# TinyMPC/tinympc-matlab

Hardware: AMD Instinct MI355X
Metric: ADMM iterations/s, batched quadrotor nx=12 nu=4 N=50 (instance-iterations/s, whole job) (higher is better)
Workload: dtype f64

## Files before the change

### __graft_entry__.py

```python
from __future__ import annotations

import hashlib
import importlib.util
import os
import re
import shutil
import subprocess
import sys

ROOT = os.path.dirname(os.path.abspath(__file__))
if ROOT not in sys.path:
    sys.path.insert(0, ROOT)
PKG_DIR = os.path.join(ROOT, "tinympc-matlab_amd")
PKG_NAME = "tinympc_matlab_amd"
CSRC = os.path.join(PKG_DIR, "csrc")
HIP_LIB = os.path.join(PKG_DIR, "libtinympc_hip.so")
ORACLE_DIR = os.path.join(ROOT, "oracle")
REFERENCE_SRC = "/root/reference/src/codegen_src"

HIP_SOURCES = ["tinympc_kernels.hip", "tinympc_precompute_rows.hip", "tinympc_solve.hip", "tinympc_solve_b.hip", "tinympc_solve_fam.hip", "tinympc_solve_adapt.hip", "tinympc_imod_a.hip", "tinympc_ifam_a.hip", "tinympc_solve_c.hip", "tinympc_solve_d.hip", "tinympc_solve_dr.hip", "tinympc_lean_d.hip", "tinympc_lstart_d.hip", "tinympc_ltrim_d.hip", "tinympc_solve_dw.hip", "tinympc_solve_dx.hip", "tinympc_jit.hip", "tinympc_solve_m.hip", "tinympc_precompute_large.hip", "tinympc_handle.hip", "tinympc_plan.hip", "tinympc_session.hip", "tinympc_capi.hip",
               "tinympc_codegen.hip"]
HIP_LINTED = ["tinympc_precompute_rows.hip", "tinympc_solve.hip", "tinympc_solve_b.hip", "tinympc_solve_fam.hip", "tinympc_solve_adapt.hip", "tinympc_imod_a.hip", "tinympc_ifam_a.hip",
              "tinympc_solve_c.hip", "tinympc_solve_d.hip", "tinympc_solve_dr.hip", "tinympc_lean_d.hip", "tinympc_lstart_d.hip", "tinympc_ltrim_d.hip", "tinympc_solve_dw.hip", "tinympc_solve_dx.hip"]
JIT_EMBEDDED = ["tinympc_device.h", "tinympc_sweep.h", "tinympc_fam_red.h", "tinympc_solve_d_chain.h", "tinympc_solve_dw_chain.h", "tinympc_solve_dx_chain.h",
                "tinympc_solve_e_common.h", "tinympc_solve_dwide.h", "tinympc_solve_d.hip", "tinympc_solve_dw.hip", "tinympc_solve_dx.hip", "tinympc_solve_e.hip",
                "tinympc_solve_f.hip"]
_ROCKET = ["-DTINY_JIT_NX=6", "-DTINY_JIT_NU=3", "-DTINY_JIT_N=100", "-DTINY_JIT_CT=0", "-DTINY_JIT_FAM=1"]
_ROCKET_FAM = ["-DTINY_JIT_E_NROUND=1", "-DTINY_JIT_E_NCONE=2", "-DTINY_JIT_E_CONES={0,0,2},{0,6,8}", "-DTINY_JIT_E_NLX=1", "-DTINY_JIT_E_NLU=0"]
HIP_BUILTINS = [
    ("k_builtin_e_rocket100", "tinympc_solve_e.hip",
     _ROCKET + ["-DTINY_JIT_E_WPG=8", "-DTINY_JIT_E_WPS=2", "-DTINY_JIT_E_S=13"] + _ROCKET_FAM +
     ["-DTINY_JIT_E_GC_LDS=0", "-DTINY_JIT_E_GL_LDS=0", "-DTINY_JIT_E_LX_LDS=0", "-DTINY_JIT_E_KFAM=1", "-DTINY_JIT_E_DREG=1"]),
    ("k_builtin_f_rocket100", "tinympc_solve_f.hip", _ROCKET + ["-DTINY_JIT_F_WPG=4", "-DTINY_JIT_F_S=7"] + _ROCKET_FAM + ["-DTINY_JIT_F_KFAM=1"]),
    ("k_builtin_f_rocket100_session", "tinympc_solve_f.hip", _ROCKET + ["-DTINY_JIT_F_WPG=4", "-DTINY_JIT_F_S=7"] + _ROCKET_FAM + ["-DTINY_JIT_F_KFAM=1", "-DTINY_JIT_F_SESSION=1"]),
]
_NO_FAM = ["-DTINY_JIT_E_NROUND=0", "-DTINY_JIT_E_NCONE=0", "-DTINY_JIT_E_CONES={-1,0,0}", "-DTINY_JIT_E_NLX=0", "-DTINY_JIT_E_NLU=0"]
for _name, _nx, _nu, _N, _wpg, _S in (("cartpole20", 4, 1, 20, 2, 3), ("quadrotor50", 12, 4, 50, 4, 4)):
    for _suffix, _ct, _extra in (("", 1, []), ("_var", 0, []), ("_session", 0, ["-DTINY_JIT_F_SESSION=1"])):
        HIP_BUILTINS.append(("k_builtin_f_%s%s" % (_name, _suffix), "tinympc_solve_f.hip",
                             ["-DTINY_JIT_NX=%d" % _nx, "-DTINY_JIT_NU=%d" % _nu, "-DTINY_JIT_N=%d" % _N, "-DTINY_JIT_CT=%d" % _ct, "-DTINY_JIT_FAM=0",
                              "-DTINY_JIT_F_WPG=%d" % _wpg, "-DTINY_JIT_F_S=%d" % _S] + _NO_FAM + _extra))
HIP_BUILTINS_D = [("k_builtin_d_quadrotor50_models", "tinympc_solve_d.hip",
                   ["-DTINY_JIT_NX=12", "-DTINY_JIT_NU=4", "-DTINY_JIT_N=50", "-DTINY_JIT_VREG=49", "-DTINY_JIT_WPS=1", "-DTINY_JIT_WPG=4",
                    "-DTINY_JIT_CT=1", "-DTINY_JIT_FAM=0", "-DTINY_JIT_ADAPT=0", "-DTINY_JIT_IMOD=1"])]
ALL_BUILTINS = HIP_BUILTINS + HIP_BUILTINS_D
BUILD_DIR = os.path.join(ROOT, "build", "hip")
HIP_CFLAGS = ["--offload-arch=gfx950", "-O3", "-std=c++17", "-fPIC", "-fno-gpu-rdc",
              "-Wall", "-Wno-unused-function", "-I" + os.path.join(ROOT, "include"), "-I" + CSRC, "-I" + BUILD_DIR]
HIP_LDFLAGS = ["--offload-arch=gfx950", "-shared", "-fPIC", "-fno-gpu-rdc", "-lhiprtc"]


def load_package():
    if PKG_NAME in sys.modules:
        return sys.modules[PKG_NAME]
    spec = importlib.util.spec_from_file_location(
        PKG_NAME, os.path.join(PKG_DIR, "__init__.py"), submodule_search_locations=[PKG_DIR])
# ... 292 lines not shown
```

### tinympc-matlab_amd/csrc/tinympc_device.h

```cpp
#pragma once
#ifndef __HIPCC_RTC__
#include <hip/hip_runtime.h>
#endif

namespace tinympc {

__host__ __device__ inline size_t ops_doubles(int W, int KT) { return (size_t)2 * W * KT + 3 * W; }

__host__ __device__ inline size_t table_rows(int N) { return (size_t)N + 2; }

constexpr int V_PAD = 4;
__host__ __device__ inline size_t v_rows(int N) { return (size_t)N + 1 + 2 * V_PAD; }
__host__ __device__ inline size_t tables_doubles(int W, int N) { return 3 * table_rows(N) * W + W; }

#if defined(__HIPCC__) || defined(__HIPCC_RTC__)
__device__ __forceinline__ void host_store(double *p, double v) { __hip_atomic_store(p, v, __ATOMIC_RELAXED, __HIP_MEMORY_SCOPE_SYSTEM); }
#endif

struct PrecomputeParams {
    int nx, nu;
    union { double rho; const double *rho_sys; };
    const double *A, *B, *fdyn, *Qd, *Rd;
    double *Kinf, *Pinf, *Quu_inv, *AmBKt, *APf, *BPf;
    int *info;
// ... 267 lines not shown
    double *rho_inst;
    int batch;
    double rho;
    double *mail;
};
hipError_t launch_setup_init(const SetupInitParams &p, hipStream_t stream);
hipError_t launch_fill_bounds(double *xmin, double *xmax, size_t X, double *umin, double *umax, size_t U, double inf, hipStream_t stream);
hipError_t launch_reset_stats(int *istats, double *dstats, double *rho_inst, int batch, double rho, hipStream_t stream);
size_t lqr_scratch_doubles(int nx, int nu);
size_t precompute_large_scratch_doubles(int nx, int nu);
hipError_t launch_precompute_large(const PrecomputeParams &p, hipStream_t stream);
hipError_t launch_build_operators(const OperatorParams &p, hipStream_t stream);
hipError_t launch_build_tables(const TableParams &p, hipStream_t stream);
hipError_t launch_store_inst_refs(const InstRefStoreParams &p, hipStream_t stream);
hipError_t launch_build_inst_tables(const InstTableParams &p, hipStream_t stream);
hipError_t launch_fill_inst_models(const InstModelFillParams &p, hipStream_t stream);
hipError_t launch_store_inst_diag(const InstDiagParams &p, hipStream_t stream);
hipError_t launch_check_positive(const double *v, int n, int *flag, hipStream_t stream);
hipError_t launch_build_inst_lin(const InstLinParams &p, hipStream_t stream);
hipError_t launch_check_inst_lin(const InstLinParams &p, int *flag, hipStream_t stream);
hipError_t launch_check_ref_steps(const int *steps, int n, int delta, int *flag, hipStream_t stream);
hipError_t launch_advance_ref_steps(int *steps, int n, int delta, hipStream_t stream);
enum class SolveExt { Box, Families, Adaptive, InstRefs, InstBounds, InstModels, InstFamilies };
hipError_t launch_solve_a(const SolveParams &p, SolveExt ext, int W, int KT, size_t lds_bytes, hipStream_t stream);
hipError_t launch_solve_b(const SolveParams &p, int W, int KT, size_t lds_bytes, hipStream_t stream);
size_t solve_b_lds_bytes(int nx, int nu, int N, int W);
constexpr int WAVES_PER_GROUP_B = 4;
bool solve_d_supported(int nx, int nu, int N, bool const_tables);
hipError_t launch_solve_d(const SolveParams &p, hipStream_t stream);
hipError_t launch_solve_d_refill(const SolveParams &p, hipStream_t stream);
hipError_t launch_solve_d_lean(const SolveParams &p, hipStream_t stream);
hipError_t launch_solve_d_lean_start(const SolveParams &p, hipStream_t stream);
hipError_t launch_solve_d_lean_trim(const SolveParams &p, hipStream_t stream);
int solve_d_workgroups(int nu, int N, bool const_tables, int groups);
size_t solve_d_lds_bytes(int nu, int N, bool const_tables);
int solve_d_resident_workgroups(int wpg);
int solve_d_wavefronts_per_workgroup(int nu, int N, bool const_tables);
bool solve_dw_supported(int nx, int nu, int N, bool const_tables);
hipError_t launch_solve_dw(const SolveParams &p, hipStream_t stream);
int solve_dw_workgroups(int nu, int N, int groups);
size_t solve_dw_lds_bytes(int nu, int N);
bool solve_dx_supported(int nx, int nu, int N, bool const_tables);
hipError_t launch_solve_dx(const SolveParams &p, hipStream_t stream);
int solve_dx_workgroups(int nu, int N, int groups);
size_t solve_dx_lds_bytes(int nu, int N);
hipError_t launch_solve_c(const SolveParams &p, int W, int KT, size_t lds_bytes, hipStream_t stream);
hipError_t launch_build_chunk_tables(const ChunkTableParams &p, hipStream_t stream);
size_t f_input_table_doubles(int nu, int S);
hipError_t launch_build_f_input_tables(const ChunkTableParams &p, hipStream_t stream);
void chunk_plan(int N, int *S, int *C, int *Lc);
size_t solve_c_lds_bytes(int nx, int Lc);
size_t solve_c_lds_bytes_refs(int nx, int nu, int N, int Lc);
size_t chunk_table_doubles(int nx, int Lc);
int chunk_ks(int nx);
hipError_t launch_build_adapt(const AdaptTableParams &p, hipStream_t stream);
inline hipError_t ensure_dynamic_lds(const void *fn, size_t bytes, size_t (&cache)[16]) {
    int dev = 0;
    hipError_t e = hipGetDevice(&dev);
    if (e != hipSuccess) return e;
    if (dev >= 0 && dev < 16 && cache[dev] >= bytes) return hipSuccess;
    e = hipFuncSetAttribute(fn, hipFuncAttributeMaxDynamicSharedMemorySize, (int)bytes);
    if (e == hipSuccess && dev >= 0 && dev < 16) cache[dev] = bytes;
    return e;
}

bool solve_m_supported(int nx, int nu);
// ... 32 lines not shown
```

### tinympc-matlab_amd/csrc/tinympc_plan.hip

```cpp
#include <cstring>
#include "tinympc_handle.h"

using namespace tinympc;
using namespace tinympc::host;

namespace {

void arm_completion_flag(tinympc_solver *s, SolveParams &p) {
    if (!p.host_sol) return;
    s->session_seq += 1;
    p.host_seq = (double)s->session_seq;
    s->flag_pending = true;
}

void decide_layout_d_variants(tinympc_solver *s) {
    if (!s->layout_d) return;
    if (s->d_varying < 0 && !s->tables_const()) {
        if (s->W == 16 && !s->d_jit && solve_d_supported(s->nx, s->nu, s->N, false)) {
            s->d_varying = 1;
        } else {
            s->d_varying_jit = solve_jit_supported(s->W, s->nx, s->nu, s->N, false);
            s->d_varying = s->d_varying_jit ? 1 : 0;
        }
    }
// ... 212 lines not shown
    const bool ct = s->tables_const();
    long resident;
    if (jit) resident = solve_jit_resident_wavefronts(s->W, s->nx, s->nu, s->N, ct);
    else {
        const int wpg = solve_d_wavefronts_per_workgroup(s->nu, s->N, ct);
        resident = (long)solve_d_resident_workgroups(wpg) * wpg;
    }
    const bool reachable = s->st.abs_pri_tol > 0.0 && s->st.abs_dua_tol > 0.0;
    if ((long)s->groups <= resident) return false;
    if (!reachable && mode != 1) return false;
    return !jit || solve_jit_refill_supported(s->W, s->nx, s->nu, s->N, ct);
}

static bool lean_applies(const tinympc_solver *s, const LaunchPlan &pl) {
    if (pl.kernel != KernelId::D_COMPILED || s->W != 16 || pl.adaptive || pl.families || s->zero_copy_tick || s->st.max_iter <= 0)
        return false;
    if (pl.inst_models) return false;
    if (refill_applies(s, pl)) return false;
    const char *env = getenv("TINYMPC_LEAN");
    const int mode = env ? atoi(env) : -1;
    if (mode == 0) return false;
    if (mode == 1) return true;
    const bool reachable = s->st.abs_pri_tol > 0.0 && s->st.abs_dua_tol > 0.0;
    return s->st.check_termination != 1 || !reachable;
}
static bool lean_start_applies() {
    const char *env = getenv("TINYMPC_LEAN_START");
    return !env || atoi(env) != 0;
}
static bool lean_trim_applies() {
    const char *env = getenv("TINYMPC_LEAN_TRIM");
    return lean_start_applies() && (!env || atoi(env) != 0);
}
static const char *lean_words(const tinympc_solver *s, const LaunchPlan &pl) {
    return !lean_applies(s, pl) ? "" : lean_trim_applies() ? " lean lds-start trim" : lean_start_applies() ? " lean lds-start" : " lean";
}

int launch(tinympc_solver *s, bool timed) {
    int rc;
    s->flag_pending = false;
    if ((rc = resolve_plan(s))) return rc;
    const LaunchPlan pl = current_plan(s);
    const bool fam = pl.families, adaptive = pl.adaptive;
    if (s->inst.lin && !pl.inst_lin) {
        const char *why = s->layout_m ? "for systems with nx+nu > 64"
                          : s->inst.models ? (s->inst.rho_verb ? "with per-instance models or rho (set_model_batch / set_rho_batch); tinympc_clear_model_batch returns to the shared model and rho"
                                                               : "with per-instance models (set_model_batch); tinympc_clear_model_batch returns to the shared model")
                          : adaptive ? "with adaptive rho"
                                     : "with more cones or rounds of overlapping cones than the generic kernel holds";
        return fail(TINYMPC_ERR_UNSUPPORTED, "per-instance linear constraints (set_linear_constraints_batch) are not supported %s; "
                    "tinympc_set_linear_constraints returns to shared rows", why);
    }
    if (s->inst_tables() && !pl.inst_refs) {
        const bool r = s->inst.refs(), b = s->inst.bounds, m = s->inst.models;
        const char *what[3], *back[3];
        int n = 0;
        if (r) { what[n] = "per-instance references (set_x_ref_batch / set_u_ref_batch)"; back[n++] = "tinympc_set_x_ref / tinympc_set_u_ref return to shared references"; }
        if (b) { what[n] = "per-instance bounds (set_bound_constraints_batch)"; back[n++] = "tinympc_set_bound_constraints returns to shared bounds"; }
        if (m) {
            what[n] = s->inst.rho_verb ? "per-instance models (set_model_batch) with per-instance rho (set_rho_batch)" : "per-instance models (set_model_batch)";
            back[n++] = s->inst.rho_verb ? "tinympc_clear_model_batch returns to the shared model and rho" : "tinympc_clear_model_batch returns to the shared model";
        }
        std::string subj, way;
        for (int i = 0; i < n; ++i) {
            subj += std::string(i == 0 ? "" : i == n - 1 ? " and " : ", ") + what[i];
            way += std::string(i == 0 ? "" : ", ") + back[i];
        }
        return fail(TINYMPC_ERR_UNSUPPORTED, "%s are not supported %s; %s", subj.c_str(),
// ... 68 lines not shown
    }
    p.adapt = s->dadapt; p.rho_inst = s->drho_inst;
    if (pl.inst_lin) { p.ilin = s->inst.lrows; p.ilin_nl = s->inst.lin_nl; }
    if (pl.inst_models) p.rho_inst = s->inst.mrho;
    if (pl.inst_refs) {
        p.iref_lr = pl.kernel == KernelId::A ? s->inst.lr_rows() : s->inst.lrg;
        p.iref_pn = s->inst.pn;
        if (pl.kernel != KernelId::A) p.ibnd = s->inst.bndg;
        else if (pl.inst_bounds) p.ibnd = s->inst.bnd;
    }
    p.rho_min = s->st.adaptive_rho_min; p.rho_max = s->st.adaptive_rho_max; p.rho_clip = s->st.adaptive_rho_enable_clipping;
    const bool kernel_takes_cold = (pl.kernel == KernelId::D_COMPILED || pl.kernel == KernelId::D_JIT) && s->st.max_iter > 0;
    if (s->cold_state && !kernel_takes_cold && (rc = materialize_cold_state(s))) return rc;
    p.cold = s->cold_state ? 1 : 0;
    s->cold_state = false;
    if (s->st.max_iter > 0) s->sol_zero_pending = false;
    else if ((rc = materialize_zero_solution(s))) return rc;
    if (refill_applies(s, pl) && !p.x0_mirror && !p.u0_host && !p.host_sol) {
        if (!s->drefill && (rc = dalloc(s, &s->drefill, 1))) return rc;
        HIP_TRY(hipMemsetAsync(s->drefill, 0, sizeof(int), s->stream));
        p.refill_next = s->drefill;
    }
    if (timed) HIP_TRY(hipEventRecord(s->ev0, s->stream));
    switch (pl.kernel) {
        case KernelId::M:
            p.ctab = s->dctab;
            HIP_TRY(launch_solve_m(p, s->stream));
            break;
        case KernelId::D_JIT:
            HIP_TRY(launch_solve_jit(p, s->W, s->stream, pl.inst_models));
            break;
        case KernelId::D_COMPILED:
            if (lean_applies(s, pl) && !p.x0_mirror && !p.u0_host && !p.refill_next)
                HIP_TRY(lean_trim_applies()    ? launch_solve_d_lean_trim(p, s->stream)
                        : lean_start_applies() ? launch_solve_d_lean_start(p, s->stream)
                                               : launch_solve_d_lean(p, s->stream));
            else HIP_TRY(s->W == 64 ? launch_solve_dx(p, s->stream) : s->W == 32 ? launch_solve_dw(p, s->stream) : launch_solve_d(p, s->stream));
            break;
        case KernelId::E:
            p.ctab = s->dctab_e; p.chunk_len = s->e_chunk_len; p.chunk_count = s->e_wpg; p.chunk_levels = 1;
            HIP_TRY(launch_solve_e(p, s->fs, s->stream));
            break;
        case KernelId::F:
            p.ctab = s->dctab_f; p.ftab = s->dftab; p.chunk_len = s->f_chunk_len; p.chunk_count = s->f_chunks; p.chunk_levels = 4;
            arm_completion_flag(s, p);
            HIP_TRY(launch_solve_f(p, s->f_fs, s->stream));
            break;
        case KernelId::C:
            p.ctab = s->dctab; p.chunk_len = s->chunk_len; p.chunk_count = s->chunk_count; p.chunk_levels = s->chunk_levels;
            arm_completion_flag(s, p);
            HIP_TRY(launch_solve_c(p, s->W, s->KT, s->lds_bytes_c, s->stream));
            break;
        case KernelId::B:
            HIP_TRY(launch_solve_b(p, s->W, s->KT, s->lds_bytes, s->stream));
            break;
        case KernelId::A:
        case KernelId::FAM_A:
        case KernelId::ADAPT_A: {
            const SolveExt ext = pl.kernel == KernelId::FAM_A ? SolveExt::Families : pl.kernel == KernelId::ADAPT_A ? SolveExt::Adaptive
                                 : pl.inst_lin ? SolveExt::InstFamilies : pl.inst_models ? SolveExt::InstModels : pl.inst_bounds ? SolveExt::InstBounds : pl.inst_refs ? SolveExt::InstRefs : SolveExt::Box;
            HIP_TRY(launch_solve_a(p, ext, s->W, s->KT, s->lds_bytes_a, s->stream));
            break;
        }
    }
    if (timed) HIP_TRY(hipEventRecord(s->ev1, s->stream));
    return TINYMPC_OK;
}
// ... 87 lines not shown
```

### tinympc-matlab_amd/csrc/tinympc_solve_d.hip

```cpp
#if defined(TINY_BUILTIN) && !defined(TINY_JIT)
#define TINY_JIT 1
#endif
#ifndef TINY_JIT
#include <atomic>
#endif
#include <type_traits>

#include "tinympc_device.h"
#include "tinympc_sweep.h"

#ifndef TINY_REFILL
#if defined(TINY_JIT_REFILL) && TINY_JIT_REFILL
#define TINY_REFILL 1
#else
#define TINY_REFILL 0
#endif
#endif

#ifndef TINY_LEAN
#define TINY_LEAN 0
#endif
#if TINY_LEAN && (TINY_REFILL || defined(TINY_JIT))
#error "TINY_LEAN: compiled-in plain kernels only"
#endif
#ifndef TINY_LEAN_START
#define TINY_LEAN_START 0
#endif
#if TINY_LEAN_START && !TINY_LEAN
#error "TINY_LEAN_START: a variant of the lean kernels"
#endif
#if TINY_LEAN_START && !defined(TINY_LEAN_NO_LDS_START)
#define TINY_LDS_START 1
#else
#define TINY_LDS_START 0
#endif
#if TINY_LEAN_START && !defined(TINY_LEAN_NO_HOIST)
#define TINY_LEAN_HOIST 1
#else
#define TINY_LEAN_HOIST 0
#endif
#ifndef TINY_LEAN_TRIM
#define TINY_LEAN_TRIM 0
#endif
#if TINY_LEAN_TRIM && !(TINY_LEAN_START && TINY_LEAN_HOIST && TINY_LDS_START)
#error "TINY_LEAN_TRIM: a variant of the lean-start kernels (LDS starts and hoisted control)"
#endif
#if TINY_LEAN_TRIM && !defined(TINY_TRIM_NO_DSTORE)
#define TINY_TRIM_DSTORE 1
#define D_DUMP_DOUBLES(nu) (2 * 4 * (nu))
#else
#define TINY_TRIM_DSTORE 0
#endif

#define TINY_STR2(x) #x
#define TINY_STR(x) TINY_STR2(x)
namespace tinympc {
template <int NX, int NU>
struct DStep;
}

#ifdef TINY_JIT
#define D_NX TINY_JIT_NX
#define D_NU TINY_JIT_NU
#include "tinympc_solve_d_chain.h"
#else
#define D_NX 12
#define D_NU 4
#include "tinympc_solve_d_chain.h"
#define D_NX 4
#define D_NU 1
#include "tinympc_solve_d_chain.h"
#endif

namespace tinympc {

template <int I, int E, class F>
__device__ __forceinline__ void static_for(F &&f) {
    if constexpr (I < E) {
        f(std::integral_constant<int, I>{});
        static_for<I + 1, E>(f);
    }
}

constexpr int D_OPS_DOUBLES = 2 * 16 * 16;
// ... 378 lines not shown
    auto load_ops = [&](const double *src, double (&m)[16]) {
        if constexpr (ADAPT) {
            const double delta = rho - rho0;
            static_for<0, 16>([&](auto K) {
                constexpr int o = (K.value < NXU ? K.value : 0) * 16;
                m[K.value] = fma(delta, src[o + (sAd - sOps)], src[o]);
            });
        } else {
            static_for<0, 16>([&](auto K) { m[K.value] = src[(K.value < NXU ? K.value : 0) * 16]; });
        }
    };
    auto vget = [&](auto S) -> double {
        if constexpr (decltype(S)::value >= VL) return Vr[decltype(S)::value - VL];
        else return sVl[decltype(S)::value * 64];
    };

#ifdef TINY_CLOCK_STAMP
    const unsigned long long ck_t0 = __builtin_amdgcn_s_memtime(), ck_r0 = __builtin_amdgcn_s_memrealtime();
#endif
#ifdef TINY_D_PAD
    asm volatile(".rept " TINY_STR(TINY_D_PAD) "\n\ts_nop 0\n\t.endr" ::: "memory");
#endif
#ifdef TINY_D_LOOP_ALIGN
    asm volatile(".p2align " TINY_STR(TINY_D_LOOP_ALIGN) ::: "memory");
#endif
    const int max_iter = p.max_iter;
#if TINY_TRIM_DSTORE
    unsigned aDw = aD;
#endif
#if TINY_LEAN
    auto iteration = [&](auto LEAN_, const int it) __attribute__((always_inline)) -> bool {
#if TINY_LEAN_HOIST
        constexpr bool LEANI = decltype(LEAN_)::value != 0, CTL_ONLY = decltype(LEAN_)::value == 2, NO_CTL = LEANI && !CTL_ONLY;
#else
        constexpr bool LEANI = decltype(LEAN_)::value;
#endif
#else
    for (int it = 0; max_iter > 0; ++it) {
#endif
        const int it0 = __builtin_amdgcn_readfirstlane(it);
#if TINY_LEAN
        const bool final_round = !LEANI && it0 >= max_iter;
#elif TINY_REFILL
        const bool final_round = REFILL ? false : it0 >= max_iter;
#else
        const bool final_round = it0 >= max_iter;
#endif
#if TINY_LEAN_HOIST
        if constexpr (TWO_PER_SIMD && !CTL_ONLY) fair_share_priority<NS>(it0, simd_slot);
#else
        if constexpr (TWO_PER_SIMD) fair_share_priority<NS>(it0, simd_slot);
#endif
#if TINY_REFILL
        const bool fin = REFILL ? it_done >= max_iter : final_round;
        const bool wb = pending || (fin && active);
#elif TINY_LEAN_HOIST
        const bool wb = NO_CTL ? false : pending || (final_round && active);
#else
        const bool wb = pending || (final_round && active);
#endif
        if (TINY_RARE(__ballot(wb) != 0ull)) {
            int lane_o = lane;
            asm volatile("" : "+v"(lane_o));
            const int r_o = lane_o & 15, j_o = lane_o >> 4;
            const bool x_o = r_o < NX;
#if TINY_REFILL
// ... 160 lines not shown
            const double snew = fmin(hi0, fmax(lo0, s));
#if TINY_LEAN_HOIST
            if constexpr (LEANI) G0 = s;
            else G0 = s - snew;
#else
            G0 = s - snew;
#endif
            pri = is_x ? fabs(x0v - snew) : 0.0;
            dua = is_x ? fabs(V0 - snew) : 0.0;
            if (may && !adapt) {
                const bool bad = !((pri < p.abs_pri_tol) && (dua * rho < p.abs_dua_tol));
#if TINY_REFILL
                may = __builtin_amdgcn_readfirstlane((int)wave_may_converge_d(__ballot(bad), __ballot(REFILL ? chk : active))) != 0;
#else
                may = __builtin_amdgcn_readfirstlane((int)wave_may_converge_d(__ballot(bad), __ballot(active))) != 0;
#endif
            }
#if TINY_REFILL
            if (TINY_RARE(may) && is_x && active) gV1u[REFILL ? row_offset(cur) : (unsigned)lane] = V0;
#else
            if (TINY_RARE(may) && is_x && active) gV1u[(unsigned)lane] = V0;
#endif
            V0 = snew;
        }
        if constexpr (FAM) {
            double gcn, gln;
            (void)families(x0v, GC0, GL0, gcn, gln);
            if (is_x) {
                GC0 = gcn;
                GL0 = gln;
            }
        }
        double xcur = x0v;
        double dcur = lds_read_async<0>(aD), vcur = 0.0;
#if TINY_LEAN
        if constexpr (VL > 0 && !LEANI) vcur = lds_read_async<0>(aV);
#else
        if constexpr (VL > 0) vcur = lds_read_async<0>(aV);
#endif
        double locur = lo_c, hicur = hi_c;
        if constexpr (!CT) {
            locur = lds_read_async<W * 8>(aT);
            hicur = lds_read_async<(TOFF + W) * 8>(aT);
        }
        lds_wait_ops(m);
#if TINY_LDS_START
        double acur = 0.0;
#endif
        auto fstep = [&](auto S) {
            constexpr int q = decltype(S)::value;
            double dn = 0.0, vn = 0.0, lon = lo_c, hin = hi_c;
            if constexpr (q + 1 < NS) dn = lds_read_async<(q + 1) * DS * 8>(aD);
#if TINY_LEAN
            if constexpr (q + 1 < VL && !LEANI) vn = lds_read_async<(q + 1) * 512>(aV);
#else
            if constexpr (q + 1 < VL) vn = lds_read_async<(q + 1) * 512>(aV);
#endif
            if constexpr (!CT && q + 1 < NS) {
                lon = lds_read_async<(q + 2) * W * 8>(aT);
                hin = lds_read_async<(TOFF + (q + 2) * W) * 8>(aT);
            }
#if TINY_LDS_START
            static_assert(K0, "step 0 starts from c0");
            double an = 0.0;
            if constexpr (LEANI && q + 1 < NS) an = lds_read_issued_here<0>(aC);
#endif
            const double xprev = xcur;
            double snew_q;
#if TINY_LEAN
            if constexpr (LEANI) {
                if constexpr (q >= VL) {
                    if constexpr (K0 && q == 0) xcur = Step::fwd_reg0_nores(dcur, m, c0, locur, hicur, G[q], Vr[q - VL]);
#if TINY_LDS_START
                    else xcur = Step::fwd_reg_start(xcur, dcur, m, acur, locur, hicur, G[q], Vr[q - VL]);
#else
                    else xcur = Step::fwd_reg_nores(xcur, dcur, m, cf, locur, hicur, G[q], Vr[q - VL]);
#endif
                    snew_q = Vr[q - VL];
                } else {
                    double vnew;
                    if constexpr (K0 && q == 0) xcur = Step::fwd_lds0_nores(dcur, m, c0, locur, hicur, G[q], vnew);
#if TINY_LDS_START
                    else xcur = Step::fwd_lds_start(xcur, dcur, m, acur, locur, hicur, G[q], vnew);
#else
                    else xcur = Step::fwd_lds_nores(xcur, dcur, m, cf, locur, hicur, G[q], vnew);
#endif
                    lds_write_async<q * 512>(aV, vnew);
                    snew_q = vnew;
                }
            } else
#endif
            if constexpr (q >= VL) {
                if constexpr (K0 && q == 0) xcur = Step::fwd_reg0(dcur, m, c0, locur, hicur, G[q], Vr[q - VL], pri, dua);
                else xcur = Step::fwd_reg(xcur, dcur, m, cf, locur, hicur, G[q], Vr[q - VL], pri, dua);
                snew_q = Vr[q - VL];
            } else {
                double vnew;
                if constexpr (K0 && q == 0) xcur = Step::fwd_lds0(dcur, m, c0, locur, hicur, G[q], vcur, vnew, pri, dua);
                else xcur = Step::fwd_lds(xcur, dcur, m, cf, locur, hicur, G[q], vcur, vnew, pri, dua);
                lds_write_async<q * 512>(aV, vnew);
                snew_q = vnew;
            }
            if constexpr (ADAPT) {
                if (adapt) {
// ... 111 lines not shown
#else
            if (active) {
#endif
                snap_pri = pri;
                snap_dua = dua;
                if constexpr (ADAPT) snap_rho = rho;
                res_valid = true;
                if (conv) {
                    status = 1;
                    active = false;
                    pending = true;
                }
            }
        }

        {
            const unsigned long long wr_d = __ballot(is_u && active);
            load_ops(sMb, m);
            auto lr_of = [&](auto S) -> double {
                double base;
                if constexpr (CT) base = lr_c;
                else base = sTl[2 * TOFF + (S.value + 1) * W];
                if constexpr (FAM) base += LX[S.value];
                return base;
            };
            double px, rcur, rnext, acc;
            {
                double lrT = is_x ? pnref_lin : lr_of(std::integral_constant<int, NS - 1>{});
                if constexpr (FAM) lrT = is_x ? pnref_lin + LX[NS - 1] : lrT;
                const double lr2 = lr_of(std::integral_constant<int, NS - 2>{});
                const double lrmc2 = is_x ? lr2 + cb : cb;
                const double v1 = vget(std::integral_constant<int, NS - 1>{}), v2 = vget(std::integral_constant<int, NS - 2>{});
                double t;
                if constexpr (ADAPT) {
                    asm("v_add_f64 %[t], %[v1], -%[g1]\n\t"
                        "v_fma_f64 %[px], %[nrho], %[t], %[lrT]\n\t"
                        "v_add_f64 %[t], %[v2], -%[g2]\n\t"
                        "v_fma_f64 %[acc], %[rhom], %[t], %[lrmc]\n\t"
                        "v_fma_f64 %[rn], %[nrho], %[t], %[lr]"
                        : [t] "=&v"(t), [px] "=&v"(px), [acc] "=&v"(acc), [rn] "=&v"(rnext)
                        : [v1] "v"(v1), [g1] "v"(G[NS - 1]), [v2] "v"(v2), [g2] "v"(G[NS - 2]), [nrho] "v"(nrho_lin), [lrT] "v"(lrT),
                          [rhom] "v"(rhom_lin), [lrmc] "v"(lrmc2), [lr] "v"(lr2));
                } else if constexpr (FOLD) {
                    asm("v_add_f64 %[t], %[v1], -%[g1]\n\t"
                        "v_fma_f64 %[px], %[sc], %[t], %[lrT]\n\t"
                        "v_add_f64 %[rn], %[v2], -%[g2]\n\t"
                        "v_fma_f64 %[acc], %[rhom], %[rn], %[lrmc]"
                        : [t] "=&v"(t), [px] "=&v"(px), [acc] "=&v"(acc), [rn] "=&v"(rnext)
                        : [v1] "v"(v1), [g1] "v"(G[NS - 1]), [v2] "v"(v2), [g2] "v"(G[NS - 2]), [sc] "v"(is_x ? nrho : 1.0),
                          [lrT] "v"(is_x ? pnref : 0.0), [rhom] "v"(rhom), [lrmc] "v"(lrmc_f));
                } else {
                    asm("v_add_f64 %[t], %[v1], -%[g1]\n\t"
                        "v_fma_f64 %[px], %[nrho], %[t], %[lrT]\n\t"
                        "v_add_f64 %[t], %[v2], -%[g2]\n\t"
                        "v_fma_f64 %[acc], %[rhom], %[t], %[lrmc]\n\t"
                        "v_fma_f64 %[rn], %[nrho], %[t], %[lr]"
                        : [t] "=&v"(t), [px] "=&v"(px), [acc] "=&v"(acc), [rn] "=&v"(rnext)
                        : [v1] "v"(v1), [g1] "v"(G[NS - 1]), [v2] "v"(v2), [g2] "v"(G[NS - 2]), [nrho] "s"(nrho), [lrT] "v"(lrT),
                          [rhom] "v"(rhom), [lrmc] "v"(lrmc2), [lr] "v"(lr2));
                }
                rcur = px;
            }
            auto vreq = [&](auto S) -> double {
                if constexpr (decltype(S)::value >= VL) return Vr[decltype(S)::value - VL];
                else return lds_read_async<decltype(S)::value * 512>(aV);
            };
            double v2cur = vreq(std::integral_constant<int, (NS >= 3 ? NS - 3 : 0)>{});
            lds_wait_ops(m);
#if TINY_LEAN_HOIST
            if constexpr (LEANI) {
                asm volatile("" : "+v"(G0));
                G0 = G0 - V0;
                asm volatile("" ::"v"(G0));
            }
#endif
            static_for<0, NS - 1>([&](auto I) {
                constexpr int s = NS - 1 - I.value;
                constexpr int s2 = s >= 2 ? s - 2 : 0;
                constexpr int s3 = s >= 3 ? s - 3 : 0;
                double v2n = 0.0;
                if constexpr (s >= 2) v2n = vreq(std::integral_constant<int, s3>{});
                const double lr2 = lr_of(std::integral_constant<int, s2>{});
                const double lrmc2 = is_x ? lr2 + cb : cb;
                double a = acc, an, rn;
                if constexpr (ADAPT) Step::bwd_v(a, px, rcur, m, v2cur, G[s2], rhom_lin, lrmc2, nrho_lin, lr2, an, rn);
                else if constexpr (FOLD) Step::bwd_fold(a, px, rcur, m, v2cur, G[s2], rhom, lrmc_f, an, rn);
                else Step::bwd(a, px, rcur, m, v2cur, G[s2], rhom, lrmc2, nrho, lr2, an, rn);
#if TINY_TRIM_DSTORE
                if constexpr (NO_CTL) lds_write_async<s * DS * 8>(aDw, a);
                else lds_write_masked<s * DS * 8>(aD, a, wr_d);
#else
                lds_write_masked<s * DS * 8>(aD, a, wr_d);
#endif
                px = a;
                rcur = rnext;
                rnext = rn;
                acc = an;
                v2cur = v2n;
            });
            {
                double a = acc;
                Step::bwd_last(a, px, rcur, m);
#if TINY_TRIM_DSTORE
                if constexpr (NO_CTL) lds_write_async<0>(aDw, a);
                else lds_write_masked<0>(aD, a, wr_d);
#else
                lds_write_masked<0>(aD, a, wr_d);
#endif
            }
        }
#if TINY_LEAN
        return false;
    };
    const bool reachable = p.abs_pri_tol > 0.0 && p.abs_dua_tol > 0.0;
    const int last_check = ct > 0 ? (max_iter / ct) * ct : 0;
    for (int it = 0; max_iter > 0;) {
        int nres = max_iter + 1;
        if (ct > 0 && reachable) nres = (it / ct + 1) * ct;
        else if (last_check > it) nres = last_check;
        const int lean_end = __builtin_amdgcn_readfirstlane(nres - 1 < max_iter ? nres - 1 : max_iter);
#if TINY_LEAN_HOIST
        if (it < lean_end) {
            if (iteration(std::integral_constant<int, 2>{}, it)) break;
#if TINY_TRIM_DSTORE
            {
                const unsigned long long live = __ballot(active);
                const unsigned lm = (unsigned)(live & 1ull) | (unsigned)((live >> 15) & 2ull) | (unsigned)((live >> 30) & 4ull) | (unsigned)((live >> 45) & 8ull);
                const int first = __builtin_ctz(lm | 16u);
                const int cls = (r / NU) % 3;
                int jt = cls == 0 ? j : (j ^ 2);
                if (((lm >> jt) & 1u) == 0u) jt = first & 3;
                const unsigned dump = lds_addr(sD) + (unsigned)((jt * NU + r % NU) * 8) - (unsigned)((cls == 2 ? 2 : 1) * DS * 8);
                aDw = (is_u && active) ? aD : dump;
            }
#endif
            for (; it < lean_end; ++it) (void)iteration(std::true_type{}, it);
            if (active) it_done = __builtin_amdgcn_readfirstlane(it);
        }
        if (iteration(std::false_type{}, it)) break;
#else
        bool over = false;
        for (; it < lean_end; ++it) {
            if (iteration(std::true_type{}, it)) {
                over = true;
                break;
            }
        }
        if (over || iteration(std::false_type{}, it)) break;
#endif
        ++it;
    }
#else
    }
#endif
    lds_wait();
#ifdef TINY_CLOCK_STAMP
    const unsigned long long ck_t1 = __builtin_amdgcn_s_memtime(), ck_r1 = __builtin_amdgcn_s_memrealtime();
#endif

#if TINY_REFILL
    if constexpr (REFILL) return;
#endif
    if (inst_ok && status == 1 && r < NXU) {
        __builtin_amdgcn_fence(__ATOMIC_RELEASE, "wavefront");
        const int rows = is_x ? N : NS;
        double *const wV = p.V + ((size_t)grp * v_rows(N) + V_PAD) * 64 + lane;
        const double *const wV2 = p.V2 + ((size_t)grp * v_rows(N) + V_PAD) * 64 + lane;
        for (int kn = 0; kn < rows; ++kn) wV[kn * 64] = wV2[kn * 64];
    }

    const double res_px = group_max<W>(is_x ? snap_pri : 0.0), res_pu = group_max<W>(is_u ? snap_pri : 0.0);
    const double rho_res = ADAPT ? snap_rho : rho;
    const double res_dx = group_max<W>(is_x ? snap_dua : 0.0) * rho_res, res_du = group_max<W>(is_u ? snap_dua : 0.0) * rho_res;

#ifdef TINY_CLOCK_STAMP
    if (p.scratch && lane == 0) {
        unsigned long long *ck = reinterpret_cast<unsigned long long *>(p.scratch) + 8 * (size_t)grp;
        ck[0] = ck_t1 - ck_t0;
        ck[1] = ck_r1 - ck_r0;
        ck[2] = ck_barrier - ck_entry;
        ck[3] = ck_r0 - ck_barrier;
        ck[4] = __builtin_amdgcn_s_memrealtime() - ck_r1;
        ck[5] = ck_entry;
        ck[6] = __builtin_amdgcn_s_memrealtime();
        ck[7] = (unsigned long long)__builtin_amdgcn_s_getreg((31 << 11) | 4) | ((unsigned long long)__builtin_amdgcn_s_getreg((3 << 11) | 20) << 32);
    }
#endif
    if (inst_ok && r == 0) {
        if constexpr (ADAPT) p.rho_inst[inst] = rho;
        p.istats[inst * 2 + 0] = it_done;
        p.istats[inst * 2 + 1] = status;
        if (res_valid) {
            p.dstats[inst * 4 + 0] = res_px;
            p.dstats[inst * 4 + 1] = res_dx;
            p.dstats[inst * 4 + 2] = res_pu;
            p.dstats[inst * 4 + 3] = res_du;
        }
    }
}

#if TINY_LEAN
#if TINY_LEAN_TRIM
#define k_admm_solve_d_lean k_admm_solve_d_lean_trim
#define k_admm_solve_d_gbnd_lean k_admm_solve_d_gbnd_lean_trim
#define launch_solve_d_lean launch_solve_d_lean_trim
static_assert(d_vl(4, 50, true, 4) == 25, "quadrotor N=50: 25 slack slots in LDS with four wavefronts per workgroup");
#elif TINY_LEAN_START
#define k_admm_solve_d_lean k_admm_solve_d_lean_start
#define k_admm_solve_d_gbnd_lean k_admm_solve_d_gbnd_lean_start
#define launch_solve_d_lean launch_solve_d_lean_start
static_assert(d_vl(4, 50, true, 4) == 25, "quadrotor N=50: 25 slack slots in LDS with four wavefronts per workgroup");
#endif
template <int NX, int NU, int N, bool CT, int WPG, int VL>
__global__ void __launch_bounds__(64 * WPG) __attribute__((amdgpu_waves_per_eu(2, 2))) k_admm_solve_d_lean(const SolveParams p) {
    extern __shared__ __attribute__((aligned(16))) double smem[];
    k_admm_solve_d_body<NX, NU, N, CT, WPG, VL>(p, smem);
}
template <int NX, int NU, int N, int WPG, int VL>
__global__ void __launch_bounds__(64 * WPG) __attribute__((amdgpu_waves_per_eu(2, 2))) k_admm_solve_d_gbnd_lean(const SolveParams p) {
    extern __shared__ __attribute__((aligned(16))) double smem[];
    k_admm_solve_d_body<NX, NU, N, true, WPG, VL, false, false, true, false, false, true>(p, smem);
}

__host__ __device__ constexpr int d_wpg(int nu, int N, bool ct) { return d_vl(nu, N, ct, 4) >= 0 ? 4 : 8; }

template <int NX, int NU, int N, bool CT>
static hipError_t launch_d_one(const SolveParams &p, hipStream_t stream) {
    constexpr int WPG = d_wpg(NU, N, CT);
    constexpr int VL = d_vl(NU, N, CT, WPG);
    if constexpr (VL < 0) {
        return hipErrorInvalidValue;
    } else {
        constexpr size_t lds = d_lds_bytes(NU, N, CT, WPG, VL);
        static size_t lds_set_l[16] = {0}, lds_set_lgoal[16] = {0};
        const int wgs = (p.groups + WPG - 1) / WPG;
// ... 230 lines not shown
```

Baseline: 1.174 billion.

## Add lean-share kernel variant keeping backward-sweep values in registers across iterations

```diff
diff --git a/__graft_entry__.py b/__graft_entry__.py
--- a/__graft_entry__.py
+++ b/__graft_entry__.py
@@ -18,10 +18,10 @@
 ORACLE_DIR = os.path.join(ROOT, "oracle")
 REFERENCE_SRC = "/root/reference/src/codegen_src"
 
-HIP_SOURCES = ["tinympc_kernels.hip", "tinympc_precompute_rows.hip", "tinympc_solve.hip", "tinympc_solve_b.hip", "tinympc_solve_fam.hip", "tinympc_solve_adapt.hip", "tinympc_imod_a.hip", "tinympc_ifam_a.hip", "tinympc_solve_c.hip", "tinympc_solve_d.hip", "tinympc_solve_dr.hip", "tinympc_lean_d.hip", "tinympc_lstart_d.hip", "tinympc_ltrim_d.hip", "tinympc_solve_dw.hip", "tinympc_solve_dx.hip", "tinympc_jit.hip", "tinympc_solve_m.hip", "tinympc_precompute_large.hip", "tinympc_handle.hip", "tinympc_plan.hip", "tinympc_session.hip", "tinympc_capi.hip",
+HIP_SOURCES = ["tinympc_kernels.hip", "tinympc_precompute_rows.hip", "tinympc_solve.hip", "tinympc_solve_b.hip", "tinympc_solve_fam.hip", "tinympc_solve_adapt.hip", "tinympc_imod_a.hip", "tinympc_ifam_a.hip", "tinympc_solve_c.hip", "tinympc_solve_d.hip", "tinympc_solve_dr.hip", "tinympc_lean_d.hip", "tinympc_lstart_d.hip", "tinympc_ltrim_d.hip", "tinympc_lshare_d.hip", "tinympc_solve_dw.hip", "tinympc_solve_dx.hip", "tinympc_jit.hip", "tinympc_solve_m.hip", "tinympc_precompute_large.hip", "tinympc_handle.hip", "tinympc_plan.hip", "tinympc_session.hip", "tinympc_capi.hip",
                "tinympc_codegen.hip"]
 HIP_LINTED = ["tinympc_precompute_rows.hip", "tinympc_solve.hip", "tinympc_solve_b.hip", "tinympc_solve_fam.hip", "tinympc_solve_adapt.hip", "tinympc_imod_a.hip", "tinympc_ifam_a.hip",
-              "tinympc_solve_c.hip", "tinympc_solve_d.hip", "tinympc_solve_dr.hip", "tinympc_lean_d.hip", "tinympc_lstart_d.hip", "tinympc_ltrim_d.hip", "tinympc_solve_dw.hip", "tinympc_solve_dx.hip"]
+              "tinympc_solve_c.hip", "tinympc_solve_d.hip", "tinympc_solve_dr.hip", "tinympc_lean_d.hip", "tinympc_lstart_d.hip", "tinympc_ltrim_d.hip", "tinympc_lshare_d.hip", "tinympc_solve_dw.hip", "tinympc_solve_dx.hip"]
 JIT_EMBEDDED = ["tinympc_device.h", "tinympc_sweep.h", "tinympc_fam_red.h", "tinympc_solve_d_chain.h", "tinympc_solve_dw_chain.h", "tinympc_solve_dx_chain.h",
                 "tinympc_solve_e_common.h", "tinympc_solve_dwide.h", "tinympc_solve_d.hip", "tinympc_solve_dw.hip", "tinympc_solve_dx.hip", "tinympc_solve_e.hip",
                 "tinympc_solve_f.hip"]
diff --git a/tinympc-matlab_amd/csrc/tinympc_device.h b/tinympc-matlab_amd/csrc/tinympc_device.h
--- a/tinympc-matlab_amd/csrc/tinympc_device.h
+++ b/tinympc-matlab_amd/csrc/tinympc_device.h
@@ -323,6 +323,7 @@
 hipError_t launch_solve_d_lean(const SolveParams &p, hipStream_t stream);
 hipError_t launch_solve_d_lean_start(const SolveParams &p, hipStream_t stream);
 hipError_t launch_solve_d_lean_trim(const SolveParams &p, hipStream_t stream);
+hipError_t launch_solve_d_lean_share(const SolveParams &p, hipStream_t stream);
 int solve_d_workgroups(int nu, int N, bool const_tables, int groups);
 size_t solve_d_lds_bytes(int nu, int N, bool const_tables);
 int solve_d_resident_workgroups(int wpg);
diff --git a/tinympc-matlab_amd/csrc/tinympc_lshare_d.hip b/tinympc-matlab_amd/csrc/tinympc_lshare_d.hip
--- /dev/null
+++ b/tinympc-matlab_amd/csrc/tinympc_lshare_d.hip
@@ -0,0 +1,5 @@
+#define TINY_LEAN 1
+#define TINY_LEAN_START 1
+#define TINY_LEAN_TRIM 1
+#define TINY_LEAN_SHARE 1
+#include "tinympc_solve_d.hip"
diff --git a/tinympc-matlab_amd/csrc/tinympc_plan.hip b/tinympc-matlab_amd/csrc/tinympc_plan.hip
--- a/tinympc-matlab_amd/csrc/tinympc_plan.hip
+++ b/tinympc-matlab_amd/csrc/tinympc_plan.hip
@@ -268,8 +268,16 @@
     const char *env = getenv("TINYMPC_LEAN_TRIM");
     return lean_start_applies() && (!env || atoi(env) != 0);
 }
+static bool lean_share_applies() {
+    const char *env = getenv("TINYMPC_LEAN_SHARE");
+    return lean_trim_applies() && (!env || atoi(env) != 0);
+}
 static const char *lean_words(const tinympc_solver *s, const LaunchPlan &pl) {
-    return !lean_applies(s, pl) ? "" : lean_trim_applies() ? " lean lds-start trim" : lean_start_applies() ? " lean lds-start" : " lean";
+    return !lean_applies(s, pl)   ? ""
+           : lean_share_applies() ? " lean lds-start trim share"
+           : lean_trim_applies()  ? " lean lds-start trim"
+           : lean_start_applies() ? " lean lds-start"
+                                  : " lean";
 }
 
 int launch(tinympc_solver *s, bool timed) {
@@ -404,7 +412,8 @@
             break;
         case KernelId::D_COMPILED:
             if (lean_applies(s, pl) && !p.x0_mirror && !p.u0_host && !p.refill_next)
-                HIP_TRY(lean_trim_applies()    ? launch_solve_d_lean_trim(p, s->stream)
+                HIP_TRY(lean_share_applies()   ? launch_solve_d_lean_share(p, s->stream)
+                        : lean_trim_applies()  ? launch_solve_d_lean_trim(p, s->stream)
                         : lean_start_applies() ? launch_solve_d_lean_start(p, s->stream)
                                                : launch_solve_d_lean(p, s->stream));
             else HIP_TRY(s->W == 64 ? launch_solve_dx(p, s->stream) : s->W == 32 ? launch_solve_dw(p, s->stream) : launch_solve_d(p, s->stream));
diff --git a/tinympc-matlab_amd/csrc/tinympc_solve_d.hip b/tinympc-matlab_amd/csrc/tinympc_solve_d.hip
--- a/tinympc-matlab_amd/csrc/tinympc_solve_d.hip
+++ b/tinympc-matlab_amd/csrc/tinympc_solve_d.hip
@@ -50,6 +50,12 @@
 #define D_DUMP_DOUBLES(nu) (2 * 4 * (nu))
 #else
 #define TINY_TRIM_DSTORE 0
+#endif
+#ifndef TINY_LEAN_SHARE
+#define TINY_LEAN_SHARE 0
+#endif
+#if TINY_LEAN_SHARE && !(TINY_LEAN_TRIM && TINY_TRIM_DSTORE)
+#error "TINY_LEAN_SHARE: a variant of the trimmed lean kernels (with their dstore addresses)"
 #endif
 
 #define TINY_STR2(x) #x
@@ -494,6 +500,9 @@
     auto iteration = [&](auto LEAN_, const int it) __attribute__((always_inline)) -> bool {
 #if TINY_LEAN_HOIST
         constexpr bool LEANI = decltype(LEAN_)::value != 0, CTL_ONLY = decltype(LEAN_)::value == 2, NO_CTL = LEANI && !CTL_ONLY;
+#if TINY_LEAN_SHARE
+        constexpr bool SH_F = decltype(LEAN_)::value >= 3, SH_B = decltype(LEAN_)::value == 3;
+#endif
 #else
         constexpr bool LEANI = decltype(LEAN_)::value;
 #endif
@@ -720,7 +729,12 @@
             }
         }
         double xcur = x0v;
+#if TINY_LEAN_SHARE
+        double dcur = 0.0, vcur = 0.0;
+        if constexpr (!(SH_F && VL == 0)) dcur = lds_read_async<0>(aD);
+#else
         double dcur = lds_read_async<0>(aD), vcur = 0.0;
+#endif
 #if TINY_LEAN
         if constexpr (VL > 0 && !LEANI) vcur = lds_read_async<0>(aV);
 #else
@@ -738,7 +752,11 @@
         auto fstep = [&](auto S) {
             constexpr int q = decltype(S)::value;
             double dn = 0.0, vn = 0.0, lon = lo_c, hin = hi_c;
+#if TINY_LEAN_SHARE
+            if constexpr (q + 1 < NS && !(SH_F && q + 1 >= VL)) dn = lds_read_async<(q + 1) * DS * 8>(aD);
+#else
             if constexpr (q + 1 < NS) dn = lds_read_async<(q + 1) * DS * 8>(aD);
+#endif
 #if TINY_LEAN
             if constexpr (q + 1 < VL && !LEANI) vn = lds_read_async<(q + 1) * 512>(aV);
 #else
@@ -758,6 +776,11 @@
 #if TINY_LEAN
             if constexpr (LEANI) {
                 if constexpr (q >= VL) {
+#if TINY_LEAN_SHARE
+                    if constexpr (SH_F && K0 && q == 0) xcur = Step::fwd_reg0_nores(Vr[q - VL], m, c0, locur, hicur, G[q], Vr[q - VL]);
+                    else if constexpr (SH_F) xcur = Step::fwd_reg_start(xcur, Vr[q - VL], m, acur, locur, hicur, G[q], Vr[q - VL]);
+                    else
+#endif
                     if constexpr (K0 && q == 0) xcur = Step::fwd_reg0_nores(dcur, m, c0, locur, hicur, G[q], Vr[q - VL]);
 #if TINY_LDS_START
                     else xcur = Step::fwd_reg_start(xcur, dcur, m, acur, locur, hicur, G[q], Vr[q - VL]);
@@ -935,6 +958,27 @@
                 const double lrmc2 = is_x ? lr2 + cb : cb;
                 const double v1 = vget(std::integral_constant<int, NS - 1>{}), v2 = vget(std::integral_constant<int, NS - 2>{});
                 double t;
+#if TINY_LEAN_SHARE
+                static_assert(NVR >= 3, "the first three slots of the backward sweep are register slots");
+                if constexpr (SH_B && FOLD) {
+                    asm("v_add_f64 %[t], %[acc], -%[g1]\n\t"
+                        "v_fma_f64 %[px], %[sc], %[t], %[lrT]\n\t"
+                        "v_add_f64 %[rn], %[v2], -%[g2]\n\t"
+                        "v_fma_f64 %[acc], %[rhom], %[rn], %[lrmc]"
+                        : [t] "=&v"(t), [px] "=&v"(px), [acc] "+v"(Vr[NS - 1 - VL]), [rn] "=&v"(rnext)
+                        : [g1] "v"(G[NS - 1]), [v2] "v"(v2), [g2] "v"(G[NS - 2]), [sc] "v"(is_x ? nrho : 1.0),
+                          [lrT] "v"(is_x ? pnref : 0.0), [rhom] "v"(rhom), [lrmc] "v"(lrmc_f));
+                } else if constexpr (SH_B) {
+                    asm("v_add_f64 %[t], %[acc], -%[g1]\n\t"
+                        "v_fma_f64 %[px], %[nrho], %[t], %[lrT]\n\t"
+                        "v_add_f64 %[t], %[v2], -%[g2]\n\t"
+                        "v_fma_f64 %[acc], %[rhom], %[t], %[lrmc]\n\t"
+                        "v_fma_f64 %[rn], %[nrho], %[t], %[lr]"
+                        : [t] "=&v"(t), [px] "=&v"(px), [acc] "+v"(Vr[NS - 1 - VL]), [rn] "=&v"(rnext)
+                        : [g1] "v"(G[NS - 1]), [v2] "v"(v2), [g2] "v"(G[NS - 2]), [nrho] "s"(nrho), [lrT] "v"(lrT),
+                          [rhom] "v"(rhom), [lrmc] "v"(lrmc2), [lr] "v"(lr2));
+                } else
+#endif
                 if constexpr (ADAPT) {
                     asm("v_add_f64 %[t], %[v1], -%[g1]\n\t"
                         "v_fma_f64 %[px], %[nrho], %[t], %[lrT]\n\t"
@@ -985,6 +1029,24 @@
                 if constexpr (s >= 2) v2n = vreq(std::integral_constant<int, s3>{});
                 const double lr2 = lr_of(std::integral_constant<int, s2>{});
                 const double lrmc2 = is_x ? lr2 + cb : cb;
+#if TINY_LEAN_SHARE
+                if constexpr (SH_B && s >= VL) {
+                    constexpr bool AN_REG = s - 1 >= VL;
+                    double &an_s = Vr[AN_REG ? s - 1 - VL : 0];
+                    double an_l, rn;
+                    const double v2op = (s == 1 && AN_REG) ? rhom : v2cur;
+                    if constexpr (FOLD && AN_REG) Step::bwd_fold(Vr[s - VL], px, rcur, m, v2op, G[s2], rhom, lrmc_f, an_s, rn);
+                    else if constexpr (FOLD) Step::bwd_fold(Vr[s - VL], px, rcur, m, v2op, G[s2], rhom, lrmc_f, an_l, rn);
+                    else if constexpr (AN_REG) Step::bwd(Vr[s - VL], px, rcur, m, v2op, G[s2], rhom, lrmc2, nrho, lr2, an_s, rn);
+                    else Step::bwd(Vr[s - VL], px, rcur, m, v2op, G[s2], rhom, lrmc2, nrho, lr2, an_l, rn);
+                    if constexpr (!AN_REG) acc = an_l;
+                    px = Vr[s - VL];
+                    rcur = rnext;
+                    rnext = rn;
+                    v2cur = v2n;
+                    return;
+                }
+#endif
                 double a = acc, an, rn;
                 if constexpr (ADAPT) Step::bwd_v(a, px, rcur, m, v2cur, G[s2], rhom_lin, lrmc2, nrho_lin, lr2, an, rn);
                 else if constexpr (FOLD) Step::bwd_fold(a, px, rcur, m, v2cur, G[s2], rhom, lrmc_f, an, rn);
@@ -1001,6 +1063,10 @@
                 acc = an;
                 v2cur = v2n;
             });
+#if TINY_LEAN_SHARE
+            if constexpr (SH_B && VL == 0) Step::bwd_last(Vr[0], px, rcur, m);
+            else
+#endif
             {
                 double a = acc;
                 Step::bwd_last(a, px, rcur, m);
@@ -1037,7 +1103,19 @@
                 aDw = (is_u && active) ? aD : dump;
             }
 #endif
+#if TINY_LEAN_SHARE
+            static_for<0, NVR>([&](auto S) { Vr[S.value] = lds_read_async<(VL + S.value) * DS * 8>(aD); });
+            lds_wait();
+            static_for<0, NVR>([&](auto S) {
+                double &vr = Vr[decltype(S)::value];
+                asm volatile("" : "+v"(vr));
+            });
+            for (; it < lean_end - 1; ++it) (void)iteration(std::integral_constant<int, 3>{}, it);
+            (void)iteration(std::integral_constant<int, 4>{}, it);
+            ++it;
+#else
             for (; it < lean_end; ++it) (void)iteration(std::true_type{}, it);
+#endif
             if (active) it_done = __builtin_amdgcn_readfirstlane(it);
         }
         if (iteration(std::false_type{}, it)) break;
@@ -1103,7 +1181,12 @@
 }
 
 #if TINY_LEAN
-#if TINY_LEAN_TRIM
+#if TINY_LEAN_SHARE
+#define k_admm_solve_d_lean k_admm_solve_d_lean_share
+#define k_admm_solve_d_gbnd_lean k_admm_solve_d_gbnd_lean_share
+#define launch_solve_d_lean launch_solve_d_lean_share
+static_assert(d_vl(4, 50, true, 4) == 25, "quadrotor N=50: 25 slack slots in LDS with four wavefronts per workgroup");
+#elif TINY_LEAN_TRIM
 #define k_admm_solve_d_lean k_admm_solve_d_lean_trim
 #define k_admm_solve_d_gbnd_lean k_admm_solve_d_gbnd_lean_trim
 #define launch_solve_d_lean launch_solve_d_lean_trim
```

Result: faster. 1.189 billion (median of 6 runs) (+1.3%).
